# moxime/joint-vae

Hardware: AMD Instinct MI355X
Metric: training_images_per_sec (higher is better)
Workload: dtype f32

## Files before the change

include/jvae_hip.h:

```cpp
#ifndef JVAE_HIP_H
#define JVAE_HIP_H

#include <stddef.h>

#ifdef __cplusplus
extern "C" {
#endif

const char* jvae_version(void);

int jvae_gemm_f32(int M, int N, int K, int batch,
                  const float* A, long sAm, long sAk, long sAb,
                  const float* B, long sBk, long sBn, long sBb,
                  float* C, long sCm, long sCn, long sCb,
                  const float* bias, int bias_mode, int flags, int splitk, void* stream);

int jvae_splitk_fold_f32(const float* part, const float* bias, float* y, int S, long MN, int N, int relu, int accumulate,
                         void* stream);

typedef struct JvaeGemmDesc {
    int M, N, K, batch;
    const float* A; long sAm, sAk, sAb;
    const float* B; long sBk, sBn, sBb;
    float* C; long sCm, sCn, sCb;
    const float* bias; int bias_mode, flags, splitk;
    int want_splits; long sCsplit; int* splits;
} JvaeGemmDesc;
int jvae_gemm_group_f32(const JvaeGemmDesc* descs, int n, void* stream);

typedef struct JvaeGemmRoute {
    int variant;
    int gx, gy, gz;
// ... 352 lines not shown
```

joint-vae_amd/csrc/adam.hip:

```cpp
#include "common.h"
#include "jvae_internal.h"

namespace {

__global__ __launch_bounds__(256) void sqnorm_kernel(const float* __restrict__ g, long n, float* __restrict__ partial) {
    __shared__ float red[17];
    float s = 0.f;
    const long n4 = n >> 2;
    for (long i = (long)blockIdx.x * blockDim.x + threadIdx.x; i < n4; i += (long)gridDim.x * blockDim.x) {
        const f32x4 v = reinterpret_cast<const f32x4*>(g)[i];
        s += v[0] * v[0] + v[1] * v[1] + v[2] * v[2] + v[3] * v[3];
    }
    if (blockIdx.x == 0)
        for (long i = (n4 << 2) + threadIdx.x; i < n; i += blockDim.x) s += g[i] * g[i];
    s = block_sum(s, red);
    if (threadIdx.x == 0) partial[blockIdx.x] = s;
}

__global__ __launch_bounds__(256) void sqnorm_fold_kernel(const float* __restrict__ partial, int nblocks, float* acc, int reset) {
    __shared__ float red[17];
    float s = 0.f;
    for (int i = threadIdx.x; i < nblocks; i += 256) s += partial[i];
    s = block_sum(s, red);
    if (threadIdx.x == 0) *acc = (reset ? 0.f : *acc) + s;
}

struct AdamP {
    float* p; const float* g; float* m; float* v; long n;
    float lr_over_bc1, b1, b2, eps, wd, inv_sqrt_bc2, max_norm;
    const float* sqnorm; int* flag;
    const float* hyper;
};

__global__ void adam_hyper_kernel(float* hyper) {
    if (threadIdx.x != 0 || blockIdx.x != 0) return;
    const double step = (double)hyper[3] + 1.0;
    hyper[3] = (float)step;
    const double bc1 = 1.0 - pow((double)hyper[1], step), bc2 = 1.0 - pow((double)hyper[2], step);
    hyper[4] = (float)((double)hyper[0] / bc1);
    hyper[5] = (float)(1.0 / sqrt(bc2));
}

__device__ __forceinline__ float adam1(float p, float g, float& m, float& v, const AdamP& a, float coef) {
    g = fmaf(g, coef, a.wd * p);
    m = a.b1 * m + (1.f - a.b1) * g;
    v = a.b2 * v + (1.f - a.b2) * g * g;
    const float denom = sqrtf(v) * a.inv_sqrt_bc2 + a.eps;
    return p - a.lr_over_bc1 * (m / denom);
}

__global__ __launch_bounds__(256) void adam_kernel(AdamP a) {
    if (a.hyper) { a.lr_over_bc1 = a.hyper[4]; a.inv_sqrt_bc2 = a.hyper[5]; a.b1 = a.hyper[1]; a.b2 = a.hyper[2]; }
    float coef = 1.f;
    if (a.max_norm > 0.f && a.sqnorm) coef = fminf(1.f, a.max_norm / (sqrtf(a.sqnorm[0]) + 1e-6f));
    bool bad = false;
    const long n4 = a.n >> 2;
    for (long i = (long)blockIdx.x * blockDim.x + threadIdx.x; i < n4; i += (long)gridDim.x * blockDim.x) {
        f32x4 p = reinterpret_cast<f32x4*>(a.p)[i];
        const f32x4 g = reinterpret_cast<const f32x4*>(a.g)[i];
        f32x4 m = reinterpret_cast<f32x4*>(a.m)[i], v = reinterpret_cast<f32x4*>(a.v)[i];
#pragma unroll
        for (int j = 0; j < 4; ++j) {
            float mj = m[j], vj = v[j];
            p[j] = adam1(p[j], g[j], mj, vj, a, coef);
            m[j] = mj; v[j] = vj;
            bad |= !isfinite(p[j]);
        }
        reinterpret_cast<f32x4*>(a.p)[i] = p;
        reinterpret_cast<f32x4*>(a.m)[i] = m;
        reinterpret_cast<f32x4*>(a.v)[i] = v;
    }
    if (blockIdx.x == 0)
        for (long i = (n4 << 2) + threadIdx.x; i < a.n; i += blockDim.x) {
            float mj = a.m[i], vj = a.v[i];
            const float pn = adam1(a.p[i], a.g[i], mj, vj, a, coef);
            a.p[i] = pn; a.m[i] = mj; a.v[i] = vj;
            bad |= !isfinite(pn);
        }
    if (a.flag && __any(bad) && (threadIdx.x & 63) == 0) atomicOr(a.flag, 1);
}

__global__ __launch_bounds__(256) void sgd_kernel(float* __restrict__ p, const float* __restrict__ g, float* __restrict__ buf,
                                                  long n, float lr, float mu, int nesterov, float wd, int first,
                                                  float max_norm, const float* __restrict__ sqnorm, int* __restrict__ flag) {
    float coef = 1.f;
    if (max_norm > 0.f && sqnorm) coef = fminf(1.f, max_norm / (sqrtf(sqnorm[0]) + 1e-6f));
    bool bad = false;
    for (long i = (long)blockIdx.x * blockDim.x + threadIdx.x; i < n; i += (long)gridDim.x * blockDim.x) {
        const float pi = p[i];
        float d = fmaf(wd, pi, coef * g[i]);
        if (mu != 0.f) {
            const float b = first ? d : fmaf(mu, buf[i], d);
            buf[i] = b;
            d = nesterov ? fmaf(mu, b, d) : b;
        }
        const float pn = pi - lr * d;
        p[i] = pn;
        bad |= !isfinite(pn);
    }
    if (flag && __any(bad) && (threadIdx.x & 63) == 0) atomicOr(flag, 1);
}

// ... 9 lines not shown
}

inline bool al16(const void* p) { return (reinterpret_cast<uintptr_t>(p) & 15) == 0; }

}

extern "C" {

size_t jvae_sqnorm_workspace_bytes(void) { return sizeof(float) * 8192; }

int jvae_sqnorm_accum_f32(const float* g, long n, float* acc, int reset, void* ws, size_t ws_bytes, void* stream) {
    if (!acc || n < 0 || (n > 0 && !g)) return JVAE_EINVAL;
    hipStream_t st = (hipStream_t)stream;
    if (n == 0) {
        if (reset) {
            hipError_t e = hipMemsetAsync(acc, 0, sizeof(float), st);
            if (e != hipSuccess) return (int)e;
        }
        return 0;
    }
    if (!al16(g)) return JVAE_EINVAL;
    if (!ws || ws_bytes < jvae_sqnorm_workspace_bytes()) return JVAE_EWORKSPACE;
    const int blocks = grid_for(n / 4);
    hipLaunchKernelGGL(sqnorm_kernel, dim3(blocks), dim3(256), 0, st, g, n, (float*)ws);
    JVAE_LAUNCH_CHECK();
    hipLaunchKernelGGL(sqnorm_fold_kernel, dim3(1), dim3(256), 0, st, (const float*)ws, blocks, acc, reset);
    JVAE_LAUNCH_CHECK();
    return 0;
}

int jvae_clip_scale_f32(float* g, long n, const float* sqnorm, float max_norm, void* stream) {
    if (!g || !sqnorm || n < 0 || !(max_norm > 0.f)) return JVAE_EINVAL;
    if (n == 0) return 0;
    hipLaunchKernelGGL(clip_scale_kernel, dim3(grid_for(n)), dim3(256), 0, (hipStream_t)stream, g, n, sqnorm, max_norm);
    JVAE_LAUNCH_CHECK();
    return 0;
}

int jvae_adam_step_f32(float* p, const float* g, float* m, float* v, long n,
                       float lr, float beta1, float beta2, float eps, float weight_decay, long step,
                       float max_norm, const float* sqnorm, int* nonfinite_flag, void* stream) {
    if (n < 0 || step < 1) return JVAE_EINVAL;
    if (n == 0) return 0;
    if (!p || !g || !m || !v) return JVAE_EINVAL;
    if (!al16(p) || !al16(g) || !al16(m) || !al16(v)) return JVAE_EINVAL;
    AdamP a;
    a.p = p; a.g = g; a.m = m; a.v = v; a.n = n;
    const double bc1 = 1.0 - pow((double)beta1, (double)step), bc2 = 1.0 - pow((double)beta2, (double)step);
    a.lr_over_bc1 = (float)((double)lr / bc1);
    a.inv_sqrt_bc2 = (float)(1.0 / sqrt(bc2));
    a.b1 = beta1; a.b2 = beta2; a.eps = eps; a.wd = weight_decay; a.max_norm = max_norm;
    a.sqnorm = sqnorm; a.flag = nonfinite_flag; a.hyper = nullptr;
    hipLaunchKernelGGL(adam_kernel, dim3(grid_for(n / 4)), dim3(256), 0, (hipStream_t)stream, a);
    JVAE_LAUNCH_CHECK();
    return 0;
}

int jvae_adam_step_dev_f32(float* p, const float* g, float* m, float* v, long n, float* hyper, int advance,
                           float eps, float weight_decay, float max_norm, const float* sqnorm, int* nonfinite_flag,
                           void* stream) {
    if (n < 0 || !hyper) return JVAE_EINVAL;
    hipStream_t st = (hipStream_t)stream;
    if (advance) {
        hipLaunchKernelGGL(adam_hyper_kernel, dim3(1), dim3(64), 0, st, hyper);
        JVAE_LAUNCH_CHECK();
    }
    if (n == 0) return 0;
    if (!p || !g || !m || !v) return JVAE_EINVAL;
    if (!al16(p) || !al16(g) || !al16(m) || !al16(v)) return JVAE_EINVAL;
    AdamP a;
    a.p = p; a.g = g; a.m = m; a.v = v; a.n = n;
    a.lr_over_bc1 = 0.f; a.inv_sqrt_bc2 = 0.f; a.b1 = 0.f; a.b2 = 0.f;
    a.eps = eps; a.wd = weight_decay; a.max_norm = max_norm;
    a.sqnorm = sqnorm; a.flag = nonfinite_flag; a.hyper = hyper;
    hipLaunchKernelGGL(adam_kernel, dim3(grid_for(n / 4)), dim3(256), 0, st, a);
    JVAE_LAUNCH_CHECK();
    return 0;
}

int jvae_sgd_step_f32(float* p, const float* g, float* buf, long n, float lr, float momentum, int nesterov,
                      float weight_decay, int first_step, float max_norm, const float* sqnorm, int* nonfinite_flag,
                      void* stream) {
    if (n < 0 || momentum < 0.f || (nesterov && momentum <= 0.f)) return JVAE_EINVAL;
    if (n == 0) return 0;
    if (!p || !g || (momentum != 0.f && !buf)) return JVAE_EINVAL;
    hipLaunchKernelGGL(sgd_kernel, dim3(grid_for(n)), dim3(256), 0, (hipStream_t)stream, p, g, buf, n, lr, momentum, nesterov,
                       weight_decay, first_step, max_norm, sqnorm, nonfinite_flag);
    JVAE_LAUNCH_CHECK();
    return 0;
}

const char* jvae_version(void) { return "jvae_hip 0.1 (gfx950)"; }

}
```

joint-vae_amd/csrc/bn.hip:

```cpp
#include <stdlib.h>
#include "bn_core.h"
#include "jvae_internal.h"

namespace {

constexpr int MAX_SPLIT_F32 = 64;
typedef float f32x2 __attribute__((ext_vector_type(2)));

__global__ __launch_bounds__(256) void bn_stats_kernel(const float* __restrict__ x, float* __restrict__ partial,
                                                       int N, int C, int P, int nsplit, const float* __restrict__ pv) {
    __shared__ float red[17];
    const int c = blockIdx.x, s = blockIdx.y;
    const float pivot = pv ? pv[c] : x[(long)c * P];
    const ImageRange ir = image_range(N, nsplit, s);
    float s1 = 0.f, s2 = 0.f;
    bn_plane_walk(x, nullptr, nullptr, ir.nb, ir.ne, C, c, P, [&](float v, float) { const float d = v - pivot; s1 += d; s2 += d * d; });
    s1 = block_sum(s1, red);
    s2 = block_sum(s2, red);
    if (threadIdx.x == 0) {
        partial[((long)c * nsplit + s) * 2 + 0] = s1;
        partial[((long)c * nsplit + s) * 2 + 1] = s2;
    }
}

__global__ __launch_bounds__(256) void bn_apply_kernel(const float* __restrict__ x, const float* __restrict__ partial,
                                                       const float* __restrict__ gamma, const float* __restrict__ beta,
                                                       float* running_mean, float* running_var, long long* num_batches_tracked,
                                                       float* save_mean, float* save_invstd, float* __restrict__ y,
                                                       int N, int C, int P, int nsplit, int nchunk, float momentum, float eps,
                                                       int training, int relu, int ext_pivot, const float* __restrict__ pivot, int count_mult) {
    __shared__ float cs[2];
    __shared__ double dred[2][4];
    const int c = blockIdx.x, j = blockIdx.y;
    BnSums t = {0., 0.};
    if (training) t = bn_fold<BN_FOLD_BLOCK_SEQ>(partial, c, nsplit, dred);
    if (threadIdx.x == 0) {
        const float g = gamma ? gamma[c] : 1.f, b = beta ? beta[c] : 0.f;
        float mean, invstd;
        if (training) {
            const double n = (double)N * P * count_mult;
            const double pv = ext_pivot ? (pivot ? (double)pivot[c] : 0.) : (double)x[(long)c * P];
            const BnMoments m = bn_moments(t.s1, t.s2, n, pv, eps);
            if (j == 0) bn_publish(m, n, c, momentum, save_mean, save_invstd, running_mean, running_var, num_batches_tracked);
            mean = m.mean;
            invstd = m.invstd;
        } else {
            mean = running_mean[c];
            invstd = rsqrtf(running_var[c] + eps);
        }
        bn_coef(g, b, mean, invstd, &cs[0], &cs[1]);
    }
    __syncthreads();
    const float sc = cs[0], sh = cs[1];
    const ImageRange ir = image_range(N, nchunk, j);
    bn_plane_walk(x, nullptr, y, ir.nb, ir.ne, C, c, P, [&](float v, float) { return jvae_act(fmaf(v, sc, sh), relu); });
}

__global__ __launch_bounds__(256) void bn_finalize_kernel(const float* __restrict__ x, const float* __restrict__ partial,
                                                         const float* __restrict__ gamma, const float* __restrict__ beta,
                                                         float* running_mean, float* running_var, long long* num_batches_tracked,
                                                         float* save_mean, float* save_invstd,
                                                         float* __restrict__ scale, float* __restrict__ shift,
                                                         int N, int C, int P, int nsplit, float momentum, float eps,
                                                         int training, int ext_pivot, const float* __restrict__ pivot) {
    __shared__ double dred[2][4];
    const int c = blockIdx.x, l = threadIdx.x;
    const float g = gamma ? gamma[c] : 1.f, b = beta ? beta[c] : 0.f;
    float mean, invstd;
    if (training) {
        const BnSums t = bn_fold<BN_FOLD_BLOCK_PAIR>(partial, c, nsplit, dred);
        const double n = (double)N * P;
        const double pv = ext_pivot ? (pivot ? (double)pivot[c] : 0.) : (double)x[(long)c * P];
        const BnMoments m = bn_moments(t.s1, t.s2, n, pv, eps);
        if (l == 0) bn_publish(m, n, c, momentum, save_mean, save_invstd, running_mean, running_var, num_batches_tracked);
        mean = m.mean;
        invstd = m.invstd;
    } else {
        mean = running_mean[c];
        invstd = rsqrtf(running_var[c] + eps);
    }
    if (l == 0) bn_coef(g, b, mean, invstd, &scale[c], &shift[c]);
}

__global__ __launch_bounds__(256) void bn_bwd_reduce_kernel(const float* __restrict__ dy, const float* __restrict__ x,
                                                            const float* __restrict__ gamma, const float* __restrict__ beta,
                                                            const float* __restrict__ mean, const float* __restrict__ invstd,
                                                            float* __restrict__ partial, int N, int C, int P, int nsplit,
                                                            int relu, int rev) {
    __shared__ float red[17];
    const int c = blockIdx.x, s = rev ? (int)(gridDim.y - 1 - blockIdx.y) : (int)blockIdx.y;
    const float neg = relu == JVAE_ACT_LEAKY ? JVAE_LEAKY_SLOPE : 0.f;
    const float mu = mean[c], is = invstd[c];
    const float g_ = gamma ? gamma[c] : 1.f, b_ = beta ? beta[c] : 0.f;
    float sc, sh;
    bn_coef(g_, b_, mu, is, &sc, &sh);
    const ImageRange ir = image_range(N, nsplit, s);
    f32x2 acc = 0.f;
    bn_plane_walk(x, dy, nullptr, ir.nb, ir.ne, C, c, P, [&](float xv, float g) {
        if (relu && !(fmaf(xv, sc, sh) > 0.f)) g *= neg;
        acc += f32x2{g, g * ((xv - mu) * is)};
    });
    float s1 = acc[0], s2 = acc[1];
    s1 = block_sum(s1, red);
    s2 = block_sum(s2, red);
// ... 132 lines not shown
    return bn_fwd_impl(x, gamma, beta, running_mean, running_var, num_batches_tracked, y, save_mean, save_invstd,
                       N, C, P, momentum, eps, training, relu, nullptr, 0, nullptr, 1, ws, ws_bytes, stream);
}

int jvae_bn_fwd_ext_f32(const float* x, const float* gamma, const float* beta,
                        float* running_mean, float* running_var, long long* num_batches_tracked,
                        float* y, float* save_mean, float* save_invstd,
                        int N, int C, int P, float momentum, float eps, int training, int relu,
                        const float* ext_stats, int ext_nsplit, const float* ext_pivot,
                        void* ws, size_t ws_bytes, void* stream) {
    return bn_fwd_impl(x, gamma, beta, running_mean, running_var, num_batches_tracked, y, save_mean, save_invstd,
                       N, C, P, momentum, eps, training, relu, ext_stats, ext_nsplit, ext_pivot, 1, ws, ws_bytes, stream);
}

int jvae_bn_finalize_f32(const float* x, const float* gamma, const float* beta,
                         float* running_mean, float* running_var, long long* num_batches_tracked,
                         float* save_mean, float* save_invstd, float* scale, float* shift,
                         int N, int C, int P, float momentum, float eps, int training,
                         const float* ext_stats, int ext_nsplit, const float* ext_pivot,
                         void* ws, size_t ws_bytes, void* stream) {
    if (!x || !scale || !shift || N <= 0 || C <= 0 || P <= 0) return JVAE_EINVAL;
    hipStream_t st = (hipStream_t)stream;
    BnStatsSrc src;
    const int rc = bn_stats_source(ws, ws_bytes, jvae_bn_workspace_bytes(C), N, training, ext_stats, ext_nsplit, save_mean, save_invstd,
                                   running_mean, running_var, pick_split(N, C, P), [&](int ns) {
        hipLaunchKernelGGL(bn_stats_kernel, dim3(C, ns), dim3(256), 0, st, x, (float*)ws, N, C, P, ns, (const float*)nullptr);
    }, &src);
    if (rc != 0) return rc;
    hipLaunchKernelGGL(bn_finalize_kernel, dim3(C), dim3(256), 0, st, x, src.partial, gamma, beta, running_mean, running_var,
                       num_batches_tracked, save_mean, save_invstd, scale, shift, N, C, P, src.nsplit, momentum, eps, training,
                       src.ext, ext_pivot);
    JVAE_LAUNCH_CHECK();
    return 0;
}

int jvae_bn_bwd_f32(const float* dy, const float* x, const float* gamma, const float* beta,
                    const float* save_mean, const float* save_invstd,
                    float* dx, float* dgamma, float* dbeta, int accumulate,
                    int N, int C, int P, int relu, void* ws, size_t ws_bytes, void* stream) {
    if (!dy || !x || !save_mean || !save_invstd || !dx || N < 0 || C <= 0 || P <= 0) return JVAE_EINVAL;
    if (ws_bytes < jvae_bn_workspace_bytes(C) || !ws) return JVAE_EWORKSPACE;
    if (N == 0) return 0;
    hipStream_t st = (hipStream_t)stream;
    float* partial = (float*)ws;
    const int ns = pick_split(N, C, P);
    const int order = 1;
    relu = jvae_act_kind(relu);
    hipLaunchKernelGGL(bn_bwd_reduce_kernel, dim3(C, ns), dim3(256), 0, st, dy, x, gamma, beta, save_mean, save_invstd,
                       partial, N, C, P, ns, relu, order & 1);
    JVAE_LAUNCH_CHECK();
    const int nc = pick_chunk(N, C, P);
// ... 85 lines not shown
```

joint-vae_amd/csrc/bn_core.h:

```cpp
#pragma once
#include <type_traits>
#include "common.h"

__device__ __forceinline__ void bn_coef(float g, float b, float mean, float invstd, float* sc, float* sh) {
    *sc = g * invstd;
    *sh = b - mean * (g * invstd);
}

enum BnFold { BN_FOLD_THREAD, BN_FOLD_WAVE, BN_FOLD_BLOCK_SEQ, BN_FOLD_BLOCK_PAIR };
struct BnSums { double s1, s2; };
template <BnFold SHAPE>
__device__ __forceinline__ BnSums bn_fold(const float* __restrict__ partial, int c, int nsplit, double (*dred)[4] = nullptr) {
    constexpr int step = SHAPE == BN_FOLD_THREAD ? 1 : (SHAPE == BN_FOLD_WAVE ? 64 : 256);
    BnSums t = {0., 0.};
    for (int s = SHAPE == BN_FOLD_THREAD ? 0 : (int)threadIdx.x; s < nsplit; s += step) {
        t.s1 += (double)partial[((long)c * nsplit + s) * 2 + 0];
        t.s2 += (double)partial[((long)c * nsplit + s) * 2 + 1];
    }
    if constexpr (SHAPE != BN_FOLD_THREAD) {
#pragma unroll
        for (int o = 32; o > 0; o >>= 1) { t.s1 += __shfl_xor(t.s1, o, 64); t.s2 += __shfl_xor(t.s2, o, 64); }
    }
    if constexpr (SHAPE == BN_FOLD_BLOCK_SEQ || SHAPE == BN_FOLD_BLOCK_PAIR) {
        if ((threadIdx.x & 63) == 0) { dred[0][threadIdx.x >> 6] = t.s1; dred[1][threadIdx.x >> 6] = t.s2; }
        __syncthreads();
        if constexpr (SHAPE == BN_FOLD_BLOCK_SEQ) {
            t.s1 = dred[0][0] + dred[0][1] + dred[0][2] + dred[0][3];
            t.s2 = dred[1][0] + dred[1][1] + dred[1][2] + dred[1][3];
        } else {
            t.s1 = (dred[0][0] + dred[0][1]) + (dred[0][2] + dred[0][3]);
            t.s2 = (dred[1][0] + dred[1][1]) + (dred[1][2] + dred[1][3]);
        }
    }
    return t;
}

struct BnMoments { float mean, invstd; double var; };
__device__ __forceinline__ BnMoments bn_moments(double s1, double s2, double n, double pv, float eps) {
    BnMoments m;
    const double dm = s1 / n;
    m.var = s2 / n - dm * dm;
    if (m.var < 0.) m.var = 0.;
    m.mean = (float)(pv + dm);
    m.invstd = (float)(1.0 / sqrt(m.var + (double)eps));
    return m;
}
__device__ __forceinline__ void bn_publish(const BnMoments& m, double n, int c, float momentum, float* save_mean, float* save_invstd,
                                           float* running_mean, float* running_var, long long* num_batches_tracked) {
    save_mean[c] = m.mean;
    save_invstd[c] = m.invstd;
    if (running_mean) running_mean[c] = (1.f - momentum) * running_mean[c] + momentum * m.mean;
    if (running_var) {
        const float unbiased = (float)(n > 1. ? m.var * n / (n - 1.) : m.var);
        running_var[c] = (1.f - momentum) * running_var[c] + momentum * unbiased;
    }
    if (c == 0 && num_batches_tracked) *num_batches_tracked += 1;
}
// ... 70 lines not shown
```

joint-vae_amd/csrc/conv_generic.hip:

```cpp
#include "common.h"
#include "jvae_internal.h"

namespace {

__global__ __launch_bounds__(256) void unfold_kernel(const float* __restrict__ xb, float* __restrict__ col,
                                                     ConvGeom g, int n0, int nimg, long sn, long sk, long sq,
                                                     int kfast) {
    const int Kd = g.Cb * g.KH * g.KW, Ps = g.Hs * g.Ws;
    const long total = (long)nimg * Kd * Ps;
    for (long i = (long)blockIdx.x * blockDim.x + threadIdx.x; i < total; i += (long)gridDim.x * blockDim.x) {
        int n, k, q;
        if (kfast) { k = (int)(i % Kd); long r = i / Kd; n = (int)(r % nimg); q = (int)(r / nimg); }
        else       { q = (int)(i % Ps); long r = i / Ps; k = (int)(r % Kd);  n = (int)(r / Kd); }
        const int kw = k % g.KW, kh = (k / g.KW) % g.KH, cb = k / (g.KW * g.KH);
        const int hs = q / g.Ws, ws = q % g.Ws;
        const int hb = hs * g.S + kh - g.P, wb = ws * g.S + kw - g.P;
        float v = 0.f;
        if (hb >= 0 && hb < g.Hb && wb >= 0 && wb < g.Wb)
            v = xb[(((long)(n0 + n) * g.Cb + cb) * g.Hb + hb) * g.Wb + wb];
        col[(long)n * sn + (long)k * sk + (long)q * sq] = v;
    }
}

template <bool KFAST>
// ... 47 lines not shown
                }
            }
            xb[(((long)(n0 + n) * g.Cb + cb) * g.Hb + hb) * g.Wb + wb] = acc;
            continue;
        }
        for (int kh = 0; kh < g.KH; ++kh) {
            const int th = hb + g.P - kh;
            if (th < 0 || th % g.S) continue;
            const int hs = th / g.S;
            if (hs >= g.Hs) continue;
            for (int kw = 0; kw < g.KW; ++kw) {
                const int tw = wb + g.P - kw;
                if (tw < 0 || tw % g.S) continue;
                const int ws = tw / g.S;
                if (ws >= g.Ws) continue;
                const int k = (cb * g.KH + kh) * g.KW + kw;
                acc += col[(long)n * sn + (long)k * sk + (long)(hs * g.Ws + ws) * sq];
            }
        }
        xb[(((long)(n0 + n) * g.Cb + cb) * g.Hb + hb) * g.Wb + wb] = acc;
    }
}

__global__ __launch_bounds__(256) void channel_sum_kernel(const float* __restrict__ t, float* __restrict__ partial,
                                                          int N, int C, int P, int nsplit) {
    __shared__ float red[17];
    const int c = blockIdx.x, sp = blockIdx.y;
    const ImageRange ir = image_range(N, nsplit, sp);
    const int nb = ir.nb, ne = ir.ne;
    float s = 0.f;
    if ((P & 3) == 0) {
        const int P4 = P >> 2;
        const long cnt = (long)(ne - nb) * P4;
        for (long i = threadIdx.x; i < cnt; i += blockDim.x) {
            const long n = nb + i / P4, q = i % P4;
            const f32x4 v = *reinterpret_cast<const f32x4*>(t + (n * C + c) * (long)P + q * 4);
            s += (v[0] + v[1]) + (v[2] + v[3]);
        }
    } else {
        const long cnt = (long)(ne - nb) * P;
        for (long i = threadIdx.x; i < cnt; i += blockDim.x) {
            const long n = nb + i / P, q = i % P;
            s += t[(n * C + c) * (long)P + q];
        }
    }
    s = block_sum(s, red);
    if (threadIdx.x == 0) partial[(long)c * nsplit + sp] = s;
}

__global__ void channel_fold_kernel(const float* __restrict__ partial, float* __restrict__ out, int C, int nsplit,
                                    int accumulate) {
    const int c = blockIdx.x * blockDim.x + threadIdx.x;
    if (c >= C) return;
    float s = 0.f;
    for (int k = 0; k < nsplit; ++k) s += partial[(long)c * nsplit + k];
    out[c] = (accumulate ? out[c] : 0.f) + s;
}

inline int fold_slab_images(const ConvGeom& g) {
    const long per = (long)g.Cb * g.Hb * g.Wb;
    long n = ((1L << 31) - 1) / (per > 0 ? per : 1);
    if (const char* e = getenv("JVAE_FOLD_SLAB")) { const long v = atol(e); if (v > 0 && v < n) n = v; }
    return (int)(n < 1 ? 1 : (n > g.N ? (g.N > 0 ? g.N : 1) : n));
}

inline int grid_for(long total) {
    long b = (total + 255) / 256;
    return (int)(b > 8192 ? 8192 : (b < 1 ? 1 : b));
}

inline int grid_for4(long total4) {
    long b = (total4 + 255) / 256;
    return (int)(b > 16384 ? 16384 : (b < 1 ? 1 : b));
}

int launch_unfold(const float* xb, float* col, const ConvGeom& g, int n0, int nimg, bool kfast, hipStream_t st) {
    const long Kd = (long)g.Cb * g.KH * g.KW, Ps = (long)g.Hs * g.Ws, total = (long)nimg * Kd * Ps;
    const bool vec = total < (1L << 31) && (kfast ? Kd % 4 == 0 : g.Ws % 4 == 0) && ((uintptr_t)col & 15) == 0;
    if (vec && kfast)
// ... 196 lines not shown
    return 0;
}

size_t jvae_channel_sum_ws_bytes(int C) { return sizeof(float) * (size_t)(C > 0 ? C : 1) * 64; }

int jvae_channel_sum(const float* t, float* out, int N, int C, int P, int accumulate, float* ws, size_t ws_bytes,
                     hipStream_t st) {
    if (C <= 0) return 0;
    if (N <= 0) {
        if (!accumulate) {
            hipError_t e = hipMemsetAsync(out, 0, sizeof(float) * (size_t)C, st);
            if (e != hipSuccess) return (int)e;
        }
        return 0;
    }
    if (!ws || ws_bytes < jvae_channel_sum_ws_bytes(C)) return JVAE_EWORKSPACE;
    long work = (long)N * P;
    int ns = (int)(work / 4096);
    const int cap = (1024 + C - 1) / C;
    if (ns > cap) ns = cap;
    if (ns > 64) ns = 64;
    if (ns > N) ns = N;
    if (ns < 1) ns = 1;
    hipLaunchKernelGGL(channel_sum_kernel, dim3(C, ns), dim3(256), 0, st, t, ws, N, C, P, ns);
    JVAE_LAUNCH_CHECK();
    hipLaunchKernelGGL(channel_fold_kernel, dim3(cdiv(C, 64)), dim3(64), 0, st, (const float*)ws, out, C, ns, accumulate);
    JVAE_LAUNCH_CHECK();
    return 0;
}
```

joint-vae_amd/csrc/jvae_internal.h:

```cpp
#pragma once
#include <hip/hip_runtime.h>
#include <type_traits>
#include "common.h"

int jvae_gemm_launch(int M, int N, int K, int batch,
                     const float* A, long sAm, long sAk, long sAb,
                     const float* B, long sBk, long sBn, long sBb,
                     float* C, long sCm, long sCn, long sCb,
                     const float* bias, int bias_mode, int flags, int splitk, hipStream_t st);

int jvae_gemm_launch_ex(int M, int N, int K, int batch,
                        const float* A, long sAm, long sAk, long sAb,
                        const float* B, long sBk, long sBn, long sBb,
                        float* C, long sCm, long sCn, long sCb,
                        const float* bias, int bias_mode, int bias_div, int flags, int splitk, hipStream_t st);

int jvae_splitk_fold_qn(const float* part, const float* bias, float* y, int S, int N, int Cs, int Ps, hipStream_t st);
int jvae_splitk_fold(const float* part, const float* bias, float* y, int S, long MN, int N, int relu, int accumulate,
                     hipStream_t st, int bias_div = 1);

int jvae_gemm_launch_part(int M, int N, int K, int batch,
                          const float* A, long sAm, long sAk, long sAb,
                          const float* B, long sBk, long sBn, long sBb,
                          float* part, long sCm, long sCn, long sCb, long sCsplit, int want_splits, int* splits,
// ... 10 lines not shown
}
template <class K>
inline int jvae_aff_lds_attr(bool& done, int bytes, K&& kernel) {
    for (int inst = 0; inst < 3 && !done; ++inst) {
        hipError_t e = hipSuccess;
        jvae_with_aff(inst, [&](auto A) {
            e = hipFuncSetAttribute(reinterpret_cast<const void*>(kernel(A)), hipFuncAttributeMaxDynamicSharedMemorySize, bytes);
        });
        if (e != hipSuccess) return (int)e;
    }
    done = true;
    return 0;
}

struct ConvGeom {
    int N;
    int Cb, Hb, Wb;
    int Cs, Hs, Ws;
    int KH, KW, S, P;
};

int jvae_wgrad_slab_reduce(const float* slab, float* dw, int G, int Ca, int Cb, int accumulate, int swapflip, hipStream_t st,
                           int tapmajor = 0, int taps = 25);
```

joint-vae_amd/jvae_hip/lib.py:

```python
import ctypes
import os
from ctypes import c_char_p, c_float, c_int, c_long, c_longlong, c_size_t, c_void_p, POINTER

import torch

_HERE = os.path.dirname(os.path.abspath(__file__))
LIB_PATH = os.environ.get('JVAE_HIP_LIB') or os.path.join(_HERE, 'libjvae_hip.so')

_lib = None

P = c_void_p


class GemmDesc(ctypes.Structure):
    _fields_ = ([('M', c_int), ('N', c_int), ('K', c_int), ('batch', c_int)]
                + [('A', P), ('sAm', c_long), ('sAk', c_long), ('sAb', c_long)]
                + [('B', P), ('sBk', c_long), ('sBn', c_long), ('sBb', c_long)]
                + [('C', P), ('sCm', c_long), ('sCn', c_long), ('sCb', c_long)]
                + [('bias', P), ('bias_mode', c_int), ('flags', c_int), ('splitk', c_int)]
                + [('want_splits', c_int), ('sCsplit', c_long), ('splits', POINTER(c_int))])


class FoldDesc(ctypes.Structure):
    _fields_ = [('part', P), ('bias', P), ('y', P), ('S', c_int), ('MN', c_long), ('N', c_int), ('relu', c_int),
                ('accumulate', c_int)]


class GemmRoute(ctypes.Structure):
    _fields_ = [(n, c_int) for n in ('variant', 'gx', 'gy', 'gz', 'slices', 'kchunk', 'vecA', 'vecB', 'lds')]


_SIGS = {
    'jvae_version': (c_char_p, []),
    'jvae_gemm_route': (c_int, [POINTER(GemmDesc), POINTER(GemmRoute)]),
    'jvae_gemm_variant_name': (c_char_p, [c_int]),
    'jvae_gemm_f32': (c_int, [c_int] * 4 + [P, c_long, c_long, c_long] * 3 + [P, c_int, c_int, c_int, P]),
    'jvae_splitk_fold_f32': (c_int, [P, P, P, c_int, c_long, c_int, c_int, c_int, P]),
    'jvae_gemm_group_f32': (c_int, [POINTER(GemmDesc), c_int, P]),
    'jvae_splitk_fold_group_f32': (c_int, [POINTER(FoldDesc), c_int, P]),
    'jvae_conv2d_workspace_bytes': (c_size_t, [c_int] * 11),
    'jvae_conv2d_set_split_bf16': (c_int, [c_int]),
    'jvae_conv2d_set_split_shape16': (c_int, [c_int]),
    'jvae_conv2d_out_shape': (c_int, [c_int] * 8 + [POINTER(c_int), POINTER(c_int)]),
    'jvae_conv2d_route': (c_int, [c_int] * 17 + [POINTER(c_int), POINTER(c_int), POINTER(c_size_t), POINTER(c_int), POINTER(c_int)]),
    'jvae_conv2d_kernel_name': (c_char_p, [c_int]),
    'jvae_conv2d_fwd_f32': (c_int, [P, P, P, P] + [c_int] * 11 + [P, c_size_t, P]),
    'jvae_conv2d_stats_splits': (c_int, [c_int] * 11),
    'jvae_conv2d_fwd_stats_f32': (c_int, [P, P, P, P, P, POINTER(c_int)] + [c_int] * 11 + [P, c_size_t, P]),
    'jvae_conv2d_dgrad_f32': (c_int, [P, P, P] + [c_int] * 11 + [P, c_size_t, P]),
    'jvae_conv2d_wgrad_f32': (c_int, [P, P, P, P, c_int] + [c_int] * 11 + [P, c_size_t, P]),
    'jvae_b8_pack_f32': (c_int, [P, P, c_int, c_int, c_long, P]),
    'jvae_b8_unpack_f32': (c_int, [P, P, c_int, c_int, c_long, c_int, P]),
    'jvae_conv2d_native_b8': (c_int, [c_int] * 11),
    'jvae_conv2d_workspace_bytes_b8': (c_size_t, [c_int] * 11),
    'jvae_conv2d_stats_splits_b8': (c_int, [c_int] * 11),
    'jvae_conv2d_fwd_b8': (c_int, [P, P, P, P, c_int, P, POINTER(c_int)] + [c_int] * 11 + [P, c_size_t, P]),
# ... 238 lines not shown
```

Measured before the change: 143,900.

## Fold split reductions in-launch via last-arriver tickets to drop finalize kernels

After: 143,800 (median of 2 runs). About the same (-0.0%).

```diff
diff --git a/include/jvae_hip.h b/include/jvae_hip.h
--- a/include/jvae_hip.h
+++ b/include/jvae_hip.h
@@ -8,6 +8,9 @@
 #endif
 
 const char* jvae_version(void);
+
+int jvae_set_inlaunch_fold(int on);
+int jvae_get_inlaunch_fold(void);
 
 int jvae_gemm_f32(int M, int N, int K, int batch,
                   const float* A, long sAm, long sAk, long sAb,
diff --git a/joint-vae_amd/csrc/adam.hip b/joint-vae_amd/csrc/adam.hip
--- a/joint-vae_amd/csrc/adam.hip
+++ b/joint-vae_amd/csrc/adam.hip
@@ -1,10 +1,10 @@
 #include "common.h"
 #include "jvae_internal.h"
+#include "last_arriver.h"
 
 namespace {
 
-__global__ __launch_bounds__(256) void sqnorm_kernel(const float* __restrict__ g, long n, float* __restrict__ partial) {
-    __shared__ float red[17];
+__device__ __forceinline__ float sqnorm_block(const float* __restrict__ g, long n, float* red) {
     float s = 0.f;
     const long n4 = n >> 2;
     for (long i = (long)blockIdx.x * blockDim.x + threadIdx.x; i < n4; i += (long)gridDim.x * blockDim.x) {
@@ -13,23 +13,50 @@
     }
     if (blockIdx.x == 0)
         for (long i = (n4 << 2) + threadIdx.x; i < n; i += blockDim.x) s += g[i] * g[i];
+    return block_sum(s, red);
+}
+
+template <class Load>
+__device__ __forceinline__ void sqnorm_fold(Load load, int nblocks, float* acc, int reset, float* red) {
+    float s = 0.f;
+    for (int i0 = threadIdx.x; i0 < nblocks; i0 += 256 * 8) {
+        float v[8];
+#pragma unroll
+        for (int k = 0; k < 8; ++k) v[k] = i0 + 256 * k < nblocks ? load(i0 + 256 * k) : 0.f;
+#pragma unroll
+        for (int k = 0; k < 8; ++k)
+            if (i0 + 256 * k < nblocks) s += v[k];
+    }
     s = block_sum(s, red);
+    if (threadIdx.x == 0) *acc = (reset ? 0.f : *acc) + s;
+}
+
+__global__ __launch_bounds__(256) void sqnorm_kernel(const float* __restrict__ g, long n, float* __restrict__ partial) {
+    __shared__ float red[17];
+    const float s = sqnorm_block(g, n, red);
     if (threadIdx.x == 0) partial[blockIdx.x] = s;
 }
 
 __global__ __launch_bounds__(256) void sqnorm_fold_kernel(const float* __restrict__ partial, int nblocks, float* acc, int reset) {
     __shared__ float red[17];
-    float s = 0.f;
-    for (int i = threadIdx.x; i < nblocks; i += 256) s += partial[i];
-    s = block_sum(s, red);
-    if (threadIdx.x == 0) *acc = (reset ? 0.f : *acc) + s;
+    sqnorm_fold([=](int i) { return partial[i]; }, nblocks, acc, reset, red);
+}
+
+__global__ __launch_bounds__(256) void sqnorm_inlaunch_kernel(const float* __restrict__ g, long n, float* partial, float* acc, int reset,
+                                                              int word) {
+    __shared__ float red[17];
+    const float s = sqnorm_block(g, n, red);
+    if (threadIdx.x == 0) la_store(partial + blockIdx.x, s);
+    if (!last_arriver_many(word, red)) return;
+    sqnorm_fold([=](int i) { return la_load(partial + i); }, (int)gridDim.x, acc, reset, red);
 }
 
 struct AdamP {
     float* p; const float* g; float* m; float* v; long n;
     float lr_over_bc1, b1, b2, eps, wd, inv_sqrt_bc2, max_norm;
     const float* sqnorm; int* flag;
-    const float* hyper;
+    float* hyper;
+    int advance, word;
 };
 
 __global__ void adam_hyper_kernel(float* hyper) {
@@ -50,7 +77,17 @@
 }
 
 __global__ __launch_bounds__(256) void adam_kernel(AdamP a) {
-    if (a.hyper) { a.lr_over_bc1 = a.hyper[4]; a.inv_sqrt_bc2 = a.hyper[5]; a.b1 = a.hyper[1]; a.b2 = a.hyper[2]; }
+    __shared__ float hs[3];
+    if (a.hyper && a.advance) {
+        if (threadIdx.x == 0) {
+            const double step = (double)a.hyper[3] + 1.0;
+            const double bc1 = 1.0 - pow((double)a.hyper[1], step), bc2 = 1.0 - pow((double)a.hyper[2], step);
+            hs[0] = (float)((double)a.hyper[0] / bc1);
+            hs[1] = (float)(1.0 / sqrt(bc2));
+        }
+        __syncthreads();
+        a.lr_over_bc1 = hs[0]; a.inv_sqrt_bc2 = hs[1]; a.b1 = a.hyper[1]; a.b2 = a.hyper[2];
+    } else if (a.hyper) { a.lr_over_bc1 = a.hyper[4]; a.inv_sqrt_bc2 = a.hyper[5]; a.b1 = a.hyper[1]; a.b2 = a.hyper[2]; }
     float coef = 1.f;
     if (a.max_norm > 0.f && a.sqnorm) coef = fminf(1.f, a.max_norm / (sqrtf(a.sqnorm[0]) + 1e-6f));
     bool bad = false;
@@ -78,6 +115,11 @@
             bad |= !isfinite(pn);
         }
     if (a.flag && __any(bad) && (threadIdx.x & 63) == 0) atomicOr(a.flag, 1);
+    if (a.hyper && a.advance && last_arriver_many(a.word, &hs[2]) && threadIdx.x == 0) {
+        a.hyper[3] = (float)((double)a.hyper[3] + 1.0);
+        a.hyper[4] = a.lr_over_bc1;
+        a.hyper[5] = a.inv_sqrt_bc2;
+    }
 }
 
 __global__ __launch_bounds__(256) void sgd_kernel(float* __restrict__ p, const float* __restrict__ g, float* __restrict__ buf,
@@ -133,6 +175,12 @@
     if (!al16(g)) return JVAE_EINVAL;
     if (!ws || ws_bytes < jvae_sqnorm_workspace_bytes()) return JVAE_EWORKSPACE;
     const int blocks = grid_for(n / 4);
+    const int word = jvae_ticket_block(st, la_many_words(blocks));
+    if (word >= 0) {
+        hipLaunchKernelGGL(sqnorm_inlaunch_kernel, dim3(blocks), dim3(256), 0, st, g, n, (float*)ws, acc, reset, word);
+        JVAE_LAUNCH_CHECK();
+        return 0;
+    }
     hipLaunchKernelGGL(sqnorm_kernel, dim3(blocks), dim3(256), 0, st, g, n, (float*)ws);
     JVAE_LAUNCH_CHECK();
     hipLaunchKernelGGL(sqnorm_fold_kernel, dim3(1), dim3(256), 0, st, (const float*)ws, blocks, acc, reset);
@@ -161,7 +209,7 @@
     a.lr_over_bc1 = (float)((double)lr / bc1);
     a.inv_sqrt_bc2 = (float)(1.0 / sqrt(bc2));
     a.b1 = beta1; a.b2 = beta2; a.eps = eps; a.wd = weight_decay; a.max_norm = max_norm;
-    a.sqnorm = sqnorm; a.flag = nonfinite_flag; a.hyper = nullptr;
+    a.sqnorm = sqnorm; a.flag = nonfinite_flag; a.hyper = nullptr; a.advance = 0; a.word = 0;
     hipLaunchKernelGGL(adam_kernel, dim3(grid_for(n / 4)), dim3(256), 0, (hipStream_t)stream, a);
     JVAE_LAUNCH_CHECK();
     return 0;
@@ -172,18 +220,18 @@
                            void* stream) {
     if (n < 0 || !hyper) return JVAE_EINVAL;
     hipStream_t st = (hipStream_t)stream;
-    if (advance) {
+    if (n > 0 && (!p || !g || !m || !v || !al16(p) || !al16(g) || !al16(m) || !al16(v))) return JVAE_EINVAL;
+    const int word = advance && n > 0 ? jvae_ticket_block(st, la_many_words(grid_for(n / 4))) : -1;
+    if (advance && word < 0) {
         hipLaunchKernelGGL(adam_hyper_kernel, dim3(1), dim3(64), 0, st, hyper);
         JVAE_LAUNCH_CHECK();
     }
     if (n == 0) return 0;
-    if (!p || !g || !m || !v) return JVAE_EINVAL;
-    if (!al16(p) || !al16(g) || !al16(m) || !al16(v)) return JVAE_EINVAL;
     AdamP a;
     a.p = p; a.g = g; a.m = m; a.v = v; a.n = n;
     a.lr_over_bc1 = 0.f; a.inv_sqrt_bc2 = 0.f; a.b1 = 0.f; a.b2 = 0.f;
     a.eps = eps; a.wd = weight_decay; a.max_norm = max_norm;
-    a.sqnorm = sqnorm; a.flag = nonfinite_flag; a.hyper = hyper;
+    a.sqnorm = sqnorm; a.flag = nonfinite_flag; a.hyper = hyper; a.advance = word >= 0; a.word = word >= 0 ? word : 0;
     hipLaunchKernelGGL(adam_kernel, dim3(grid_for(n / 4)), dim3(256), 0, st, a);
     JVAE_LAUNCH_CHECK();
     return 0;
diff --git a/joint-vae_amd/csrc/bn.hip b/joint-vae_amd/csrc/bn.hip
--- a/joint-vae_amd/csrc/bn.hip
+++ b/joint-vae_amd/csrc/bn.hip
@@ -1,25 +1,32 @@
 #include <stdlib.h>
 #include "bn_core.h"
 #include "jvae_internal.h"
+#include "last_arriver.h"
 
 namespace {
 
 constexpr int MAX_SPLIT_F32 = 64;
 typedef float f32x2 __attribute__((ext_vector_type(2)));
 
-__global__ __launch_bounds__(256) void bn_stats_kernel(const float* __restrict__ x, float* __restrict__ partial,
-                                                       int N, int C, int P, int nsplit, const float* __restrict__ pv) {
-    __shared__ float red[17];
+__device__ __forceinline__ void bn_stats_block(const float* __restrict__ x, int N, int C, int P, int nsplit, const float* __restrict__ pv,
+                                               float* red, float* s1o, float* s2o) {
     const int c = blockIdx.x, s = blockIdx.y;
     const float pivot = pv ? pv[c] : x[(long)c * P];
     const ImageRange ir = image_range(N, nsplit, s);
     float s1 = 0.f, s2 = 0.f;
     bn_plane_walk(x, nullptr, nullptr, ir.nb, ir.ne, C, c, P, [&](float v, float) { const float d = v - pivot; s1 += d; s2 += d * d; });
-    s1 = block_sum(s1, red);
-    s2 = block_sum(s2, red);
+    *s1o = block_sum(s1, red);
+    *s2o = block_sum(s2, red);
+}
+
+__global__ __launch_bounds__(256) void bn_stats_kernel(const float* __restrict__ x, float* __restrict__ partial,
+                                                       int N, int C, int P, int nsplit, const float* __restrict__ pv) {
+    __shared__ float red[17];
+    float s1, s2;
+    bn_stats_block(x, N, C, P, nsplit, pv, red, &s1, &s2);
     if (threadIdx.x == 0) {
-        partial[((long)c * nsplit + s) * 2 + 0] = s1;
-        partial[((long)c * nsplit + s) * 2 + 1] = s2;
+        partial[((long)blockIdx.x * nsplit + blockIdx.y) * 2 + 0] = s1;
+        partial[((long)blockIdx.x * nsplit + blockIdx.y) * 2 + 1] = s2;
     }
 }
 
@@ -56,19 +63,19 @@
     bn_plane_walk(x, nullptr, y, ir.nb, ir.ne, C, c, P, [&](float v, float) { return jvae_act(fmaf(v, sc, sh), relu); });
 }
 
-__global__ __launch_bounds__(256) void bn_finalize_kernel(const float* __restrict__ x, const float* __restrict__ partial,
-                                                         const float* __restrict__ gamma, const float* __restrict__ beta,
-                                                         float* running_mean, float* running_var, long long* num_batches_tracked,
-                                                         float* save_mean, float* save_invstd,
-                                                         float* __restrict__ scale, float* __restrict__ shift,
-                                                         int N, int C, int P, int nsplit, float momentum, float eps,
-                                                         int training, int ext_pivot, const float* __restrict__ pivot) {
-    __shared__ double dred[2][4];
-    const int c = blockIdx.x, l = threadIdx.x;
+template <class Load>
+__device__ __forceinline__ void bn_finalize_channel(Load load, int c, const float* __restrict__ x,
+                                                    const float* __restrict__ gamma, const float* __restrict__ beta,
+                                                    float* running_mean, float* running_var, long long* num_batches_tracked,
+                                                    float* save_mean, float* save_invstd,
+                                                    float* __restrict__ scale, float* __restrict__ shift,
+                                                    int N, int P, int nsplit, float momentum, float eps,
+                                                    int training, int ext_pivot, const float* __restrict__ pivot, double (*dred)[4]) {
+    const int l = threadIdx.x;
     const float g = gamma ? gamma[c] : 1.f, b = beta ? beta[c] : 0.f;
     float mean, invstd;
     if (training) {
-        const BnSums t = bn_fold<BN_FOLD_BLOCK_PAIR>(partial, c, nsplit, dred);
+        const BnSums t = bn_fold_with<BN_FOLD_BLOCK_PAIR>(load, c, nsplit, dred);
         const double n = (double)N * P;
         const double pv = ext_pivot ? (pivot ? (double)pivot[c] : 0.) : (double)x[(long)c * P];
         const BnMoments m = bn_moments(t.s1, t.s2, n, pv, eps);
@@ -80,6 +87,39 @@
         invstd = rsqrtf(running_var[c] + eps);
     }
     if (l == 0) bn_coef(g, b, mean, invstd, &scale[c], &shift[c]);
+}
+
+__global__ __launch_bounds__(256) void bn_finalize_kernel(const float* __restrict__ x, const float* __restrict__ partial,
+                                                         const float* __restrict__ gamma, const float* __restrict__ beta,
+                                                         float* running_mean, float* running_var, long long* num_batches_tracked,
+                                                         float* save_mean, float* save_invstd,
+                                                         float* __restrict__ scale, float* __restrict__ shift,
+                                                         int N, int C, int P, int nsplit, float momentum, float eps,
+                                                         int training, int ext_pivot, const float* __restrict__ pivot) {
+    __shared__ double dred[2][4];
+    bn_finalize_channel([=](long i) { return partial[i]; }, blockIdx.x, x, gamma, beta, running_mean, running_var, num_batches_tracked,
+                        save_mean, save_invstd, scale, shift, N, P, nsplit, momentum, eps, training, ext_pivot, pivot, dred);
+}
+
+__global__ __launch_bounds__(256) void bn_stats_finalize_kernel(const float* __restrict__ x, float* partial,
+                                                               const float* __restrict__ gamma, const float* __restrict__ beta,
+                                                               float* running_mean, float* running_var, long long* num_batches_tracked,
+                                                               float* save_mean, float* save_invstd,
+                                                               float* __restrict__ scale, float* __restrict__ shift,
+                                                               int N, int C, int P, int nsplit, float momentum, float eps, int word,
+                                                               int wstride) {
+    __shared__ float red[17];
+    __shared__ double dred[2][4];
+    const int c = blockIdx.x;
+    float s1, s2;
+    bn_stats_block(x, N, C, P, nsplit, nullptr, red, &s1, &s2);
+    if (threadIdx.x == 0) {
+        la_store(partial + ((long)c * nsplit + blockIdx.y) * 2 + 0, s1);
+        la_store(partial + ((long)c * nsplit + blockIdx.y) * 2 + 1, s2);
+    }
+    if (!last_arriver(word + c * wstride, nsplit, red)) return;
+    bn_finalize_channel([=](long i) { return la_load(partial + i); }, c, x, gamma, beta, running_mean, running_var, num_batches_tracked,
+                        save_mean, save_invstd, scale, shift, N, P, nsplit, momentum, eps, 1, 0, nullptr, dred);
 }
 
 __global__ __launch_bounds__(256) void bn_bwd_reduce_kernel(const float* __restrict__ dy, const float* __restrict__ x,
@@ -258,11 +298,19 @@
     if (!x || !scale || !shift || N <= 0 || C <= 0 || P <= 0) return JVAE_EINVAL;
     hipStream_t st = (hipStream_t)stream;
     BnStatsSrc src;
+    bool folded = false;
     const int rc = bn_stats_source(ws, ws_bytes, jvae_bn_workspace_bytes(C), N, training, ext_stats, ext_nsplit, save_mean, save_invstd,
                                    running_mean, running_var, pick_split(N, C, P), [&](int ns) {
-        hipLaunchKernelGGL(bn_stats_kernel, dim3(C, ns), dim3(256), 0, st, x, (float*)ws, N, C, P, ns, (const float*)nullptr);
+        const int wstride = la_channel_stride(C, ns), word = wstride ? jvae_ticket_block(st, C * wstride) : -1;
+        folded = word >= 0;
+        if (folded)
+            hipLaunchKernelGGL(bn_stats_finalize_kernel, dim3(C, ns), dim3(256), 0, st, x, (float*)ws, gamma, beta, running_mean,
+                               running_var, num_batches_tracked, save_mean, save_invstd, scale, shift, N, C, P, ns, momentum, eps, word,
+                               wstride);
+        else
+            hipLaunchKernelGGL(bn_stats_kernel, dim3(C, ns), dim3(256), 0, st, x, (float*)ws, N, C, P, ns, (const float*)nullptr);
     }, &src);
-    if (rc != 0) return rc;
+    if (rc != 0 || folded) return rc;
     hipLaunchKernelGGL(bn_finalize_kernel, dim3(C), dim3(256), 0, st, x, src.partial, gamma, beta, running_mean, running_var,
                        num_batches_tracked, save_mean, save_invstd, scale, shift, N, C, P, src.nsplit, momentum, eps, training,
                        src.ext, ext_pivot);
diff --git a/joint-vae_amd/csrc/bn_core.h b/joint-vae_amd/csrc/bn_core.h
--- a/joint-vae_amd/csrc/bn_core.h
+++ b/joint-vae_amd/csrc/bn_core.h
@@ -9,13 +9,14 @@
 
 enum BnFold { BN_FOLD_THREAD, BN_FOLD_WAVE, BN_FOLD_BLOCK_SEQ, BN_FOLD_BLOCK_PAIR };
 struct BnSums { double s1, s2; };
-template <BnFold SHAPE>
-__device__ __forceinline__ BnSums bn_fold(const float* __restrict__ partial, int c, int nsplit, double (*dred)[4] = nullptr) {
+template <BnFold SHAPE, class Load>
+__device__ __forceinline__ BnSums bn_fold_with(Load load, int c, int nsplit, double (*dred)[4] = nullptr) {
     constexpr int step = SHAPE == BN_FOLD_THREAD ? 1 : (SHAPE == BN_FOLD_WAVE ? 64 : 256);
     BnSums t = {0., 0.};
     for (int s = SHAPE == BN_FOLD_THREAD ? 0 : (int)threadIdx.x; s < nsplit; s += step) {
-        t.s1 += (double)partial[((long)c * nsplit + s) * 2 + 0];
-        t.s2 += (double)partial[((long)c * nsplit + s) * 2 + 1];
+        const float a = load(((long)c * nsplit + s) * 2 + 0), b = load(((long)c * nsplit + s) * 2 + 1);
+        t.s1 += (double)a;
+        t.s2 += (double)b;
     }
     if constexpr (SHAPE != BN_FOLD_THREAD) {
 #pragma unroll
@@ -33,6 +34,10 @@
         }
     }
     return t;
+}
+template <BnFold SHAPE>
+__device__ __forceinline__ BnSums bn_fold(const float* __restrict__ partial, int c, int nsplit, double (*dred)[4] = nullptr) {
+    return bn_fold_with<SHAPE>([=](long i) { return partial[i]; }, c, nsplit, dred);
 }
 
 struct BnMoments { float mean, invstd; double var; };
diff --git a/joint-vae_amd/csrc/conv_generic.hip b/joint-vae_amd/csrc/conv_generic.hip
--- a/joint-vae_amd/csrc/conv_generic.hip
+++ b/joint-vae_amd/csrc/conv_generic.hip
@@ -1,5 +1,6 @@
 #include "common.h"
 #include "jvae_internal.h"
+#include "last_arriver.h"
 
 namespace {
 
@@ -93,9 +94,7 @@
     }
 }
 
-__global__ __launch_bounds__(256) void channel_sum_kernel(const float* __restrict__ t, float* __restrict__ partial,
-                                                          int N, int C, int P, int nsplit) {
-    __shared__ float red[17];
+__device__ __forceinline__ float channel_sum_block(const float* __restrict__ t, int N, int C, int P, int nsplit, float* red) {
     const int c = blockIdx.x, sp = blockIdx.y;
     const ImageRange ir = image_range(N, nsplit, sp);
     const int nb = ir.nb, ne = ir.ne;
@@ -115,17 +114,41 @@
             s += t[(n * C + c) * (long)P + q];
         }
     }
-    s = block_sum(s, red);
-    if (threadIdx.x == 0) partial[(long)c * nsplit + sp] = s;
+    return block_sum(s, red);
+}
+
+template <class Load>
+__device__ __forceinline__ void channel_fold(Load load, float* __restrict__ out, int c, int nsplit, int accumulate) {
+    float s = 0.f;
+    for (int k = 0; k < nsplit; ++k) s += load((long)c * nsplit + k);
+    out[c] = (accumulate ? out[c] : 0.f) + s;
+}
+
+__global__ __launch_bounds__(256) void channel_sum_kernel(const float* __restrict__ t, float* __restrict__ partial,
+                                                          int N, int C, int P, int nsplit) {
+    __shared__ float red[17];
+    const float s = channel_sum_block(t, N, C, P, nsplit, red);
+    if (threadIdx.x == 0) partial[(long)blockIdx.x * nsplit + blockIdx.y] = s;
 }
 
 __global__ void channel_fold_kernel(const float* __restrict__ partial, float* __restrict__ out, int C, int nsplit,
                                     int accumulate) {
     const int c = blockIdx.x * blockDim.x + threadIdx.x;
     if (c >= C) return;
-    float s = 0.f;
-    for (int k = 0; k < nsplit; ++k) s += partial[(long)c * nsplit + k];
-    out[c] = (accumulate ? out[c] : 0.f) + s;
+    channel_fold([=](long i) { return partial[i]; }, out, c, nsplit, accumulate);
+}
+
+__global__ __launch_bounds__(256) void channel_sum_inlaunch_kernel(const float* __restrict__ t, float* partial, float* __restrict__ out,
+                                                                   int N, int C, int P, int nsplit, int accumulate, int word, int wstride) {
+    __shared__ float red[17];
+    const int c = blockIdx.x;
+    const float s = channel_sum_block(t, N, C, P, nsplit, red);
+    if (threadIdx.x == 0) la_store(partial + (long)c * nsplit + blockIdx.y, s);
+    if (!last_arriver(word + c * wstride, nsplit, red) || threadIdx.x >= 64) return;
+    const float v = (int)threadIdx.x < nsplit ? la_load(partial + (long)c * nsplit + threadIdx.x) : 0.f;
+    float f = 0.f;
+    for (int k = 0; k < nsplit; ++k) f += __shfl(v, k, 64);
+    if (threadIdx.x == 0) out[c] = (accumulate ? out[c] : 0.f) + f;
 }
 
 inline int fold_slab_images(const ConvGeom& g) {
@@ -368,6 +391,13 @@
     if (ns > 64) ns = 64;
     if (ns > N) ns = N;
     if (ns < 1) ns = 1;
+    const int wstride = la_channel_stride(C, ns), word = wstride ? jvae_ticket_block(st, C * wstride) : -1;
+    if (word >= 0) {
+        hipLaunchKernelGGL(channel_sum_inlaunch_kernel, dim3(C, ns), dim3(256), 0, st, t, ws, out, N, C, P, ns, accumulate, word,
+                           wstride);
+        JVAE_LAUNCH_CHECK();
+        return 0;
+    }
     hipLaunchKernelGGL(channel_sum_kernel, dim3(C, ns), dim3(256), 0, st, t, ws, N, C, P, ns);
     JVAE_LAUNCH_CHECK();
     hipLaunchKernelGGL(channel_fold_kernel, dim3(cdiv(C, 64)), dim3(64), 0, st, (const float*)ws, out, C, ns, accumulate);
diff --git a/joint-vae_amd/csrc/jvae_internal.h b/joint-vae_amd/csrc/jvae_internal.h
--- a/joint-vae_amd/csrc/jvae_internal.h
+++ b/joint-vae_amd/csrc/jvae_internal.h
@@ -56,3 +56,7 @@
 
 int jvae_wgrad_slab_reduce(const float* slab, float* dw, int G, int Ca, int Cb, int accumulate, int swapflip, hipStream_t st,
                            int tapmajor = 0, int taps = 25);
+
+constexpr int JVAE_TICKET_WORDS = 4096;
+constexpr int JVAE_TICKET_STREAMS = 32;
+int jvae_ticket_block(hipStream_t st, int words);
diff --git a/joint-vae_amd/csrc/last_arriver.h b/joint-vae_amd/csrc/last_arriver.h
--- /dev/null
+++ b/joint-vae_amd/csrc/last_arriver.h
@@ -0,0 +1,49 @@
+#pragma once
+#include "jvae_internal.h"
+
+static __device__ unsigned jvae_ticket_word[JVAE_TICKET_STREAMS * JVAE_TICKET_WORDS];
+
+__device__ __forceinline__ void la_store(float* p, float v) { __hip_atomic_store(p, v, __ATOMIC_RELAXED, __HIP_MEMORY_SCOPE_AGENT); }
+__device__ __forceinline__ float la_load(float* p) { return __hip_atomic_load(p, __ATOMIC_RELAXED, __HIP_MEMORY_SCOPE_AGENT); }
+
+__device__ __forceinline__ bool last_arriver(int word, unsigned expected, float* slot) {
+    asm volatile("s_waitcnt vmcnt(0)" ::: "memory");
+    __syncthreads();
+    if (threadIdx.x == 0) {
+        unsigned* t = &jvae_ticket_word[word];
+        const bool last = __hip_atomic_fetch_add(t, 1u, __ATOMIC_RELAXED, __HIP_MEMORY_SCOPE_AGENT) + 1u == expected;
+        if (last) __hip_atomic_store(t, 0u, __ATOMIC_RELAXED, __HIP_MEMORY_SCOPE_AGENT);
+        *slot = last ? 1.f : 0.f;
+    }
+    __syncthreads();
+    return *slot != 0.f;
+}
+
+constexpr int JVAE_TICKET_FAN = 64, JVAE_TICKET_RUN_STRIDE = 64;
+
+inline int la_channel_stride(int C, int ns) {
+    if ((long)C * JVAE_TICKET_RUN_STRIDE <= JVAE_TICKET_WORDS) return JVAE_TICKET_RUN_STRIDE;
+    return ns <= 8 && C <= JVAE_TICKET_WORDS ? 1 : 0;
+}
+inline int la_many_words(int nblocks) { return nblocks <= JVAE_TICKET_FAN ? 1 : (1 + (nblocks + JVAE_TICKET_FAN - 1) / JVAE_TICKET_FAN) * JVAE_TICKET_RUN_STRIDE; }
+__device__ __forceinline__ bool last_arriver_many(int word, float* slot) {
+    const unsigned n = gridDim.x;
+    if (n <= (unsigned)JVAE_TICKET_FAN) return last_arriver(word, n, slot);
+    asm volatile("s_waitcnt vmcnt(0)" ::: "memory");
+    __syncthreads();
+    if (threadIdx.x == 0) {
+        const unsigned run = blockIdx.x / JVAE_TICKET_FAN, runs = (n + JVAE_TICKET_FAN - 1) / JVAE_TICKET_FAN;
+        const unsigned members = run + 1 < runs ? (unsigned)JVAE_TICKET_FAN : n - run * JVAE_TICKET_FAN;
+        unsigned* t = &jvae_ticket_word[word + (1 + run) * JVAE_TICKET_RUN_STRIDE];
+        bool last = __hip_atomic_fetch_add(t, 1u, __ATOMIC_RELAXED, __HIP_MEMORY_SCOPE_AGENT) + 1u == members;
+        if (last) {
+            __hip_atomic_store(t, 0u, __ATOMIC_RELAXED, __HIP_MEMORY_SCOPE_AGENT);
+            t = &jvae_ticket_word[word];
+            last = __hip_atomic_fetch_add(t, 1u, __ATOMIC_RELAXED, __HIP_MEMORY_SCOPE_AGENT) + 1u == runs;
+            if (last) __hip_atomic_store(t, 0u, __ATOMIC_RELAXED, __HIP_MEMORY_SCOPE_AGENT);
+        }
+        *slot = last ? 1.f : 0.f;
+    }
+    __syncthreads();
+    return *slot != 0.f;
+}
diff --git a/joint-vae_amd/csrc/last_arriver.hip b/joint-vae_amd/csrc/last_arriver.hip
--- /dev/null
+++ b/joint-vae_amd/csrc/last_arriver.hip
@@ -0,0 +1,46 @@
+#include <stdlib.h>
+#include <mutex>
+#include "jvae_internal.h"
+
+namespace {
+
+std::mutex g_mu;
+int g_on = -1;
+hipStream_t g_stream[JVAE_TICKET_STREAMS];
+int g_streams = 0;
+
+int fold_on_locked() {
+    if (g_on < 0) {
+        const char* e = getenv("JVAE_INLAUNCH_FOLD");
+        g_on = !(e && e[0] == '0' && !e[1]);
+    }
+    return g_on;
+}
+
+}
+
+int jvae_ticket_block(hipStream_t st, int words) {
+    std::lock_guard<std::mutex> lock(g_mu);
+    if (!fold_on_locked() || words > JVAE_TICKET_WORDS) return -1;
+    for (int i = 0; i < g_streams; ++i)
+        if (g_stream[i] == st) return i * JVAE_TICKET_WORDS;
+    if (g_streams == JVAE_TICKET_STREAMS) return -1;
+    g_stream[g_streams] = st;
+    return g_streams++ * JVAE_TICKET_WORDS;
+}
+
+extern "C" {
+
+int jvae_set_inlaunch_fold(int on) {
+    std::lock_guard<std::mutex> lock(g_mu);
+    const int prev = fold_on_locked();
+    g_on = on != 0;
+    return prev;
+}
+
+int jvae_get_inlaunch_fold(void) {
+    std::lock_guard<std::mutex> lock(g_mu);
+    return fold_on_locked();
+}
+
+}
diff --git a/joint-vae_amd/jvae_hip/lib.py b/joint-vae_amd/jvae_hip/lib.py
--- a/joint-vae_amd/jvae_hip/lib.py
+++ b/joint-vae_amd/jvae_hip/lib.py
@@ -32,6 +32,8 @@
 
 _SIGS = {
     'jvae_version': (c_char_p, []),
+    'jvae_set_inlaunch_fold': (c_int, [c_int]),
+    'jvae_get_inlaunch_fold': (c_int, []),
     'jvae_gemm_route': (c_int, [POINTER(GemmDesc), POINTER(GemmRoute)]),
     'jvae_gemm_variant_name': (c_char_p, [c_int]),
     'jvae_gemm_f32': (c_int, [c_int] * 4 + [P, c_long, c_long, c_long] * 3 + [P, c_int, c_int, c_int, P]),
```
